# Tomiinek/Multilingual_Text_to_Speech

Measured on NVIDIA H100. Metric: mel-frames/sec (train fwd+bwd), higher is better.
Workload: dtype bf16

## Files before the change

### multilingual_text_to_speech_b200/csrc/decoder_persist_bwd.cu

```cuda
#include <cuda_bf16.h>
#include "decoder_internal.cuh"
#include "tc_ptx.cuh"

namespace b200tts {

namespace {

constexpr int PT = 256;

__device__ __forceinline__ void ldmatrix_x4(uint32_t& r0, uint32_t& r1, uint32_t& r2, uint32_t& r3, const void* p) {
    const uint32_t addr = (uint32_t)__cvta_generic_to_shared(p);
    asm volatile("ldmatrix.sync.aligned.m8n8.x4.shared.b16 {%0,%1,%2,%3}, [%4];\n" : "=r"(r0), "=r"(r1), "=r"(r2), "=r"(r3) : "r"(addr));
}
__device__ __forceinline__ void mma_bf16(float (&c)[4], const uint32_t (&a)[4], uint32_t b0, uint32_t b1) {
    asm volatile("mma.sync.aligned.m16n8k16.row.col.f32.bf16.bf16.f32 {%0,%1,%2,%3}, {%4,%5,%6,%7}, {%8,%9}, {%0,%1,%2,%3};\n"
                 : "+f"(c[0]), "+f"(c[1]), "+f"(c[2]), "+f"(c[3])
                 : "r"(a[0]), "r"(a[1]), "r"(a[2]), "r"(a[3]), "r"(b0), "r"(b1));
}
struct NoOverlap { __device__ __forceinline__ void operator()() const {} };
template <typename Overlap = NoOverlap>
__device__ __forceinline__ bool grid_barrier(unsigned* counter, unsigned& target, unsigned nblocks, int* abort_flag, bool async_fence = false,
                                             Overlap overlap = Overlap()) {
    __shared__ int s_ok;
    __syncthreads();
    if (threadIdx.x == 0) {
        target += nblocks;
        if (async_fence) tcx::proxy_fence_global();
        asm volatile("red.release.gpu.global.add.u32 [%0], 1;" ::"l"(counter) : "memory");
    }
    overlap();
    if (threadIdx.x == 0) {
        int ok = 1;
        const long long t0 = clock64();
        unsigned polls = 0;
        for (;;) {
            unsigned v;
            asm volatile("ld.relaxed.gpu.global.u32 %0, [%1];" : "=r"(v) : "l"(counter) : "memory");
            if (v >= target) break;
            if ((++polls & 255u) == 0 && (clock64() - t0 > 4000000000ll || *reinterpret_cast<volatile int*>(abort_flag))) {
                ok = 0; *abort_flag = 1; break;
            }
        }
        asm volatile("fence.acquire.gpu;" ::: "memory");
        s_ok = ok;
    }
    __syncthreads();
    return s_ok != 0;
}

__device__ __forceinline__ void l2_prefetch(const void* p) { asm volatile("prefetch.global.L2 [%0];" ::"l"(p)); }
__device__ __forceinline__ void cp_async16(void* smem, const void* gmem) {
    asm volatile("cp.async.cg.shared.global [%0], [%1], 16;" ::"r"((uint32_t)__cvta_generic_to_shared(smem)), "l"(gmem) : "memory");
}
__device__ __forceinline__ void cp_async8(void* smem, const void* gmem) {
    asm volatile("cp.async.ca.shared.global [%0], [%1], 8;" ::"r"((uint32_t)__cvta_generic_to_shared(smem)), "l"(gmem) : "memory");
}
__device__ __forceinline__ void cp_async_wait_all() { asm volatile("cp.async.wait_all;" ::: "memory"); }
__device__ __forceinline__ void st_async_peer_f32(const float* local_smem, const uint64_t* local_bar, uint32_t peer_rank, float v) {
    uint32_t ra, rb;
    asm volatile("mapa.shared::cluster.u32 %0, %1, %2;" : "=r"(ra) : "r"((uint32_t)__cvta_generic_to_shared(local_smem)), "r"(peer_rank));
    asm volatile("mapa.shared::cluster.u32 %0, %1, %2;" : "=r"(rb) : "r"((uint32_t)__cvta_generic_to_shared(local_bar)), "r"(peer_rank));
    asm volatile("st.async.shared::cluster.mbarrier::complete_tx::bytes.b32 [%0], %1, [%2];" ::"r"(ra), "r"(__float_as_uint(v)), "r"(rb) : "memory");
}
__device__ __forceinline__ float tanh_exp(float x) { return 2.f * __fdividef(1.f, 1.f + __expf(-2.f * x)) - 1.f; }

#define BPROF_DECL long long prof_acc[8] = {0, 0, 0, 0, 0, 0, 0, 0}; long long prof_t = clock64();
#define BPROF_MARK(slot)                                                                                         \
    do {                                                                                                         \
        if (p.prof && threadIdx.x == 0) { const long long now = clock64(); prof_acc[slot] += now - prof_t; prof_t = now; } \
    } while (0)
#define BPROF_FLUSH                                                                                              \
    do {                                                                                                         \
        if (p.prof && threadIdx.x == 0)                                                                          \
            for (int k9 = 0; k9 < 8; ++k9) p.prof[(size_t)blockIdx.x * 8 + k9] = prof_acc[k9];                   \
    } while (0)

constexpr int KBA = 8;
constexpr int GLD = 33;
constexpr int NBT = 16;
constexpr int TUN = 80;
constexpr int TUN_WIDE = 96;

struct AttBwdArgs {
    int B, T, D, M, L, A, KC, NOUT, UK, UN, MT;
    const float* W; int ldw;
    const float* gates; const float* cstate;
    const float* dh_static;
    const float* dctx_static;
    const uint8_t* mask_h; const uint8_t* mask_c;
    int kind, training; float rate_h, rate_c;
    float* dgates;
    __nv_bfloat16* dgb;
    long long dgb_step; int dgb_rows;
    float* part;
    const float* q; const float* cum; const float* align; long long align_bstride;
    const float* dalign; long long dalign_bstride;
    const float* bias; const float* v; const float* Wq;
    const __nv_bfloat16* WcB;
    const __nv_bfloat16* WcB2;
    const __nv_bfloat16* memTf;
    const uint4* memFb; int M16;
    const int* lengths;
    float* dctx_tot;
    float* dq;
    float* de;
    unsigned* barrier; int* abort_flag;
    long long* prof;
};

__device__ __forceinline__ uint32_t pack2(float lo, float hi) {
    __nv_bfloat162 v = __floats2bfloat162_rn(lo, hi);
    return *reinterpret_cast<uint32_t*>(&v);
}
__device__ __forceinline__ float tanh_fast(float x) {
    float y;
    asm("tanh.approx.f32 %0, %1;" : "=f"(y) : "f"(x));
    return y;
}

template <int UNC>
__global__ void __launch_bounds__(PT, 1) att_bwd_loop_kernel(const __grid_constant__ CUtensorMap tmG, const AttBwdArgs p) {
    extern __shared__ __align__(1024) unsigned char smem_raw0[];
    unsigned char* smem_raw = reinterpret_cast<unsigned char*>((reinterpret_cast<uintptr_t>(smem_raw0) + 1023) & ~(uintptr_t)1023);
    __shared__ uint64_t full_bar[2], xb1, xb2;
    const int tid = threadIdx.x, lane = tid & 31, warp = tid >> 5;
    const int cta = blockIdx.x;
    const int kb = (cta >> 1) % KBA, nb = 2 * (cta >> 4) + (cta & 1);
    const int B = p.B, D = p.D, UK = p.UK, UN = p.UN, KROWS = 4 * UK, M = p.M, L = p.L, A = p.A;
    const int n0 = nb * UN;
    const int NKT = KROWS / 64;
    unsigned char* sW = smem_raw;
    __nv_bfloat16* As = reinterpret_cast<__nv_bfloat16*>(smem_raw + (size_t)NKT * UN * 128);
    unsigned char* extra = reinterpret_cast<unsigned char*>(As) + (size_t)NKT * 8192;
    __nv_bfloat16* sWcB = reinterpret_cast<__nv_bfloat16*>(extra);
    __nv_bfloat16* sWcB2 = sWcB + (size_t)A * 40;
    float* dcum = reinterpret_cast<float*>(sWcB2 + (size_t)32 * (A + 8));
    uint4* wqf = reinterpret_cast<uint4*>(dcum + (p.MT * 16 + 32));
    float* s_dhq = reinterpret_cast<float*>(wqf + (size_t)(A / 16) * 32);
    float* s_pbo = s_dhq + 2 * 64 * 8;
    uint8_t* s_pbm = reinterpret_cast<uint8_t*>(s_pbo + (size_t)6 * B * 8);
    float* s_rp = reinterpret_cast<float*>(s_pbm + (size_t)2 * B * 8);
    const unsigned nblocks = gridDim.x;
    const int L16 = p.MT * 16;

    for (int idx = tid; idx < KROWS * UN; idx += PT) {
        const int r = idx / UN, n = idx % UN;
        const int g = r / UK, uk = r % UK;
        float w = 0.f;
        if (n0 + n < p.NOUT) w = p.W[(size_t)(g * D + kb * UK + uk) * p.ldw + n0 + n];
        const int c = r >> 6, kc = r & 63;
        *reinterpret_cast<__nv_bfloat16*>(sW + (size_t)c * UN * 128 + n * 128 + ((((kc >> 3) ^ (n & 7))) << 4) + (kc & 7) * 2) = __float2bfloat16_rn(w);
    }
    for (int idx = tid; idx < A * 40; idx += PT) sWcB[idx] = p.WcB[idx];
    for (int idx = tid; idx < 32 * (A + 8); idx += PT) sWcB2[idx] = p.WcB2[idx];
    for (int idx = tid; idx < L16 + 32; idx += PT) dcum[idx] = 0.f;
    const int UOWN = 8;
    const bool owner = cta * UOWN < D;
    const int uo0 = cta * UOWN;
    if (owner)
        for (int idx = tid; idx < (A / 16) * 32; idx += PT) {
            const int kk = idx >> 5, g = (idx >> 2) & 7, tq = idx & 3;
            uint32_t f[4];
#pragma unroll
            for (int r2 = 0; r2 < 2; ++r2) {
                const int a = kk * 16 + 2 * tq + 8 * r2;
                const float x0 = p.Wq[(size_t)a * D + uo0 + g], x1 = p.Wq[(size_t)(a + 1) * D + uo0 + g];
                const __nv_bfloat16 h0 = __float2bfloat16_rn(x0), h1 = __float2bfloat16_rn(x1);
                __nv_bfloat162 hp; hp.x = h0; hp.y = h1;
                f[r2] = *reinterpret_cast<uint32_t*>(&hp);
                f[2 + r2] = pack2(x0 - __bfloat162float(h0), x1 - __bfloat162float(h1));
            }
            wqf[idx] = make_uint4(f[0], f[1], f[2], f[3]);
        }
    uint32_t prod_it = 0;
    if (tid == 0) { tcx::mbar_init(&xb1, 1); tcx::mbar_init(&xb2, 1); tcx::mbar_init_fence(); }
    if (tid == 0) { tcx::mbar_init(&full_bar[0], 1); tcx::mbar_init(&full_bar[1], 1); tcx::mbar_init_fence(); }
    tcx::proxy_fence_shared();
    __syncthreads();
    tcx::cluster_arrive(); tcx::cluster_wait();

    const float inv_h = 1.f / (1.f - p.rate_h), inv_c = 1.f / (1.f - p.rate_c);
    constexpr int MAXE = 3;
    float dc_reg[MAXE], dhz_reg[MAXE];
#pragma unroll
    for (int e = 0; e < MAXE; ++e) { dc_reg[e] = 0.f; dhz_reg[e] = 0.f; }
    unsigned target = 0;

    float* scr = reinterpret_cast<float*>(As);
    float* s_dctx = scr;
    float* s_w = s_dctx + ((M + 3) & ~3);
    float* s_de = s_w + L16;
    float* s_qb = s_de + L16;
    float* s_vv = s_qb + A;
    uint32_t* s_Ph = reinterpret_cast<uint32_t*>(s_vv + A);
    uint32_t* s_Pl = s_Ph + (L16 + 48);
    float* s_red = reinterpret_cast<float*>(s_Pl + (L16 + 48));
    const int hf = cta & 1, HT0 = (p.MT + 1) / 2;
    const int t_lo = hf ? HT0 : 0, t_hi = hf ? p.MT : HT0;
    const int g_lo = hf ? (HT0 - 1) * 16 : 0;
    float* s_G = s_red + 64;
    float* s_dqp = s_G + (size_t)(HT0 + 1) * 16 * GLD;
    float* s_dqx = s_dqp + 8 * A;
    float* s_dotx = s_dqx + A;
    float* s_stage = s_dotx + 4;
    uint2* s_bf = reinterpret_cast<uint2*>(s_stage + L16);
    BPROF_DECL

    const int pc = cta >> 1;
    auto pb_stage = [&](int step) {
        if (!owner || step < 0) return;
        const size_t row = (size_t)step * B;
        for (int c = tid; c < 12 * B; c += PT) {
            const int k = c / (2 * B), r = c - k * 2 * B, b = r >> 1, h4 = (r & 1) * 4;
            const float* src = k < 4 ? p.gates + (row + b) * 4 * D + (size_t)k * D : (k == 4 ? p.cstate : p.dh_static) + (row + b) * D;
            cp_async16(s_pbo + (k * B + b) * UOWN + h4, src + uo0 + h4);
        }
        if (p.training)
            for (int c = tid; c < 2 * B; c += PT) {
                const int k = c / B, b = c - k * B;
                const uint8_t* m = k ? p.mask_c : p.mask_h;
                if (m) cp_async8(s_pbm + (k * B + b) * UOWN, m + (row + b) * D + uo0);
            }
// ... 58 lines not shown
                    }
                    if (m < L16) { s_w[m] = r_w[e]; s_de[m] = r_da[e]; }
                    if (m < L16 + 48) {
                        const __nv_bfloat16 h0 = __float2bfloat16_rn(r_c0[e]), h1 = __float2bfloat16_rn(r_c1[e]);
                        __nv_bfloat162 hp; hp.x = h0; hp.y = h1;
                        s_Ph[m] = *reinterpret_cast<uint32_t*>(&hp);
                        s_Pl[m] = pack2(r_c0[e] - __bfloat162float(h0), r_c1[e] - __bfloat162float(h1));
                    }
                }
                if (tid < A) { s_qb[tid] = r_q + bias_r; s_vv[tid] = v_r; }
            }
            __syncthreads();
            for (int idx = tid; idx < p.M16 * 32; idx += PT) {
                const int kt = idx >> 5, gg = (idx >> 2) & 7, tt = idx & 3;
                const int m0 = kt * 16 + 2 * tt;
                uint2 f = make_uint2(0u, 0u);
                if (gg < 2) {
                    const float w0 = m0 < M ? s_dctx[m0] : 0.f, w1 = m0 + 1 < M ? s_dctx[m0 + 1] : 0.f;
                    const float w2 = m0 + 8 < M ? s_dctx[m0 + 8] : 0.f, w3 = m0 + 9 < M ? s_dctx[m0 + 9] : 0.f;
                    const float h0 = __bfloat162float(__float2bfloat16_rn(w0)), h1 = __bfloat162float(__float2bfloat16_rn(w1));
                    const float h2 = __bfloat162float(__float2bfloat16_rn(w2)), h3 = __bfloat162float(__float2bfloat16_rn(w3));
                    f = gg == 0 ? make_uint2(pack2(h0, h1), pack2(h2, h3)) : make_uint2(pack2(w0 - h0, w1 - h1), pack2(w2 - h2, w3 - h3));
                }
                s_bf[idx] = f;
            }
            __syncthreads();
            {
                const int g = lane >> 2, tq = lane & 3;
                for (int lt = t_lo + warp; lt < t_hi; lt += 8) {
                    float dacc[4] = {0.f, 0.f, 0.f, 0.f}, dacc2[4] = {0.f, 0.f, 0.f, 0.f};
                    if (lt * 16 < len) {
                        const uint4* fr = p.memFb + (((size_t)b * p.MT + lt) * p.M16) * 32 + lane;
                        for (int kt0 = 0; kt0 < p.M16; kt0 += KT) {
                            uint4 av[KT];
#pragma unroll
                            for (int j = 0; j < KT; ++j)
                                if (kt0 + j < p.M16) av[j] = __ldg(fr + (size_t)(kt0 + j) * 32);
                            uint32_t bfr[KT][2];
#pragma unroll
                            for (int j = 0; j < KT; ++j) {
                                bfr[j][0] = 0u; bfr[j][1] = 0u;
                                if (kt0 + j < p.M16) { const uint2 f = s_bf[(kt0 + j) * 32 + lane]; bfr[j][0] = f.x; bfr[j][1] = f.y; }
                            }
#pragma unroll
                            for (int j = 0; j < KT; j += 2) {
                                if (kt0 + j < p.M16) {
                                    const uint32_t af[4] = {av[j].x, av[j].y, av[j].z, av[j].w};
                                    mma_bf16(dacc, af, bfr[j][0], bfr[j][1]);
                                }
                                if (kt0 + j + 1 < p.M16) {
                                    const uint32_t af[4] = {av[j + 1].x, av[j + 1].y, av[j + 1].z, av[j + 1].w};
                                    mma_bf16(dacc2, af, bfr[j + 1][0], bfr[j + 1][1]);
                                }
                            }
                        }
                    }
#pragma unroll
                    for (int q4 = 0; q4 < 4; ++q4) dacc[q4] += dacc2[q4];
                    if (tq == 0) {
#pragma unroll
                        for (int rr = 0; rr < 2; ++rr) {
                            const int l = lt * 16 + g + 8 * rr;
                            float gv = 0.f;
                            if (l < len) gv = (rr ? dacc[2] + dacc[3] : dacc[0] + dacc[1]) + (last ? 0.f : dcum[l]) + s_de[l];
                            s_de[l] = gv;
                        }
                    }
                }
            }
            __syncthreads();
            float pdot = 0.f;
            for (int l = t_lo * 16 + tid; l < t_hi * 16 && l < len; l += PT) pdot = fmaf(s_w[l], s_de[l], pdot);
            pdot = block_sum(pdot, s_red);
            if (tid == 0) { tcx::mbar_expect_tx(&xb1, 4); st_async_peer_f32(s_dotx, &xb1, (uint32_t)(hf ^ 1), pdot); }
            tcx::mbar_wait(&xb1, (uint32_t)(p.T - 1 - i) & 1);
            const float dot = pdot + s_dotx[0];
            for (int l = t_lo * 16 + tid; l < t_hi * 16; l += PT) {
                const float d = l < len ? s_w[l] * (s_de[l] - dot) : 0.f;
                s_de[l] = d;
                if (l < L) p.de[((size_t)i * B + b) * L + l] = d;
            }
            __syncthreads();
            BPROF_MARK(0);
            float dqacc[16][2];
#pragma unroll
            for (int nt = 0; nt < 16; ++nt) { dqacc[nt][0] = 0.f; dqacc[nt][1] = 0.f; }
            const int g = lane >> 2, tq = lane & 3;
            for (int mt = t_lo + warp; mt < t_hi && mt < mtiles; mt += 8) {
                const int l0 = mt * 16;
                float sacc[16][4];
#pragma unroll
                for (int nt = 0; nt < 16; ++nt)
#pragma unroll
                    for (int e = 0; e < 4; ++e) sacc[nt][e] = 0.f;
#pragma unroll
                for (int ks = 0; ks < 2; ++ks) {
                    const int x = l0 + ks * 16 + g + 2 * tq;
                    uint32_t ah[4], al[4];
                    ah[0] = s_Ph[x]; ah[1] = s_Ph[x + 8]; ah[2] = s_Ph[x + 8]; ah[3] = s_Ph[x + 16];
                    al[0] = s_Pl[x]; al[1] = s_Pl[x + 8]; al[2] = s_Pl[x + 8]; al[3] = s_Pl[x + 16];
#pragma unroll
                    for (int np = 0; np < 8; ++np) {
                        uint32_t bf[4];
                        ldmatrix_x4(bf[0], bf[1], bf[2], bf[3], sWcB + (size_t)(np * 16 + (lane & 7) + ((lane >> 4) << 3)) * 40 + ks * 16 + ((lane >> 3) & 1) * 8);
                        mma_bf16(sacc[2 * np], ah, bf[0], bf[1]);
                        mma_bf16(sacc[2 * np], al, bf[0], bf[1]);
                        mma_bf16(sacc[2 * np + 1], ah, bf[2], bf[3]);
                        mma_bf16(sacc[2 * np + 1], al, bf[2], bf[3]);
                    }
                }
                const uint4* mf = reinterpret_cast<const uint4*>(p.memTf + (((size_t)b * p.MT + mt) * 32 + lane) * 64);
                const float de0 = s_de[l0 + g], de1 = s_de[l0 + g + 8];
                uint32_t dsA[16][2];
#pragma unroll
                for (int c4 = 0; c4 < 8; ++c4) {
                    const uint4 raw = mf[c4];
                    const uint32_t words[4] = {raw.x, raw.y, raw.z, raw.w};
#pragma unroll
                    for (int hf = 0; hf < 2; ++hf) {
                        const int nt = 2 * c4 + hf;
                        const float2 m01 = __bfloat1622float2(*reinterpret_cast<const __nv_bfloat162*>(&words[2 * hf]));
                        const float2 m23 = __bfloat1622float2(*reinterpret_cast<const __nv_bfloat162*>(&words[2 * hf + 1]));
                        const int a0 = nt * 8 + 2 * tq;
                        const float t0 = tanh_fast(sacc[nt][0] + s_qb[a0] + m01.x), t1 = tanh_fast(sacc[nt][1] + s_qb[a0 + 1] + m01.y);
                        const float t2 = tanh_fast(sacc[nt][2] + s_qb[a0] + m23.x), t3 = tanh_fast(sacc[nt][3] + s_qb[a0 + 1] + m23.y);
                        const float d0 = de0 * s_vv[a0] * (1.f - t0 * t0), d1 = de0 * s_vv[a0 + 1] * (1.f - t1 * t1);
                        const float d2 = de1 * s_vv[a0] * (1.f - t2 * t2), d3 = de1 * s_vv[a0 + 1] * (1.f - t3 * t3);
                        dqacc[nt][0] += d0 + d2; dqacc[nt][1] += d1 + d3;
                        dsA[nt][0] = pack2(d0, d1); dsA[nt][1] = pack2(d2, d3);
                    }
                }
                float gacc[4][4];
#pragma unroll
                for (int nt = 0; nt < 4; ++nt)
#pragma unroll
                    for (int e = 0; e < 4; ++e) gacc[nt][e] = 0.f;
#pragma unroll
                for (int j = 0; j < 8; ++j) {
                    const uint32_t af[4] = {dsA[2 * j][0], dsA[2 * j][1], dsA[2 * j + 1][0], dsA[2 * j + 1][1]};
#pragma unroll
                    for (int np = 0; np < 2; ++np) {
                        uint32_t bf[4];
                        ldmatrix_x4(bf[0], bf[1], bf[2], bf[3], sWcB2 + (size_t)(np * 16 + (lane & 7) + ((lane >> 4) << 3)) * (A + 8) + j * 16 + ((lane >> 3) & 1) * 8);
                        mma_bf16(gacc[2 * np], af, bf[0], bf[1]);
                        mma_bf16(gacc[2 * np + 1], af, bf[2], bf[3]);
                    }
                }
#pragma unroll
                for (int nt = 0; nt < 4; ++nt)
#pragma unroll
                    for (int e = 0; e < 4; ++e) s_G[(l0 - g_lo + g + 8 * (e >> 1)) * GLD + nt * 8 + 2 * tq + (e & 1)] = gacc[nt][e];
            }
            tcx::proxy_fence_shared();
            __syncthreads();
            {
                const int ht = hf ? HT0 : HT0 - 1;
                const int peer_g_lo = hf ? 0 : (HT0 - 1) * 16;
                if (tid == 0 && ht >= t_lo && ht < t_hi)
                    tcx::bulk_copy_to_peer(s_G + (size_t)(ht * 16 - peer_g_lo) * GLD, s_G + (size_t)(ht * 16 - g_lo) * GLD, 16 * GLD * 4, &xb2,
                                           (uint32_t)(hf ^ 1));
            }
#pragma unroll
            for (int nt = 0; nt < 16; ++nt)
#pragma unroll
                for (int c = 0; c < 2; ++c) {
                    float v = dqacc[nt][c];
                    v += __shfl_xor_sync(0xffffffffu, v, 4);
                    v += __shfl_xor_sync(0xffffffffu, v, 8);
                    v += __shfl_xor_sync(0xffffffffu, v, 16);
                    if (g == 0) s_dqp[warp * A + nt * 8 + 2 * tq + c] = v;
                }
            __syncthreads();
            float pdq = 0.f;
            if (tid < A) {
#pragma unroll
                for (int w8 = 0; w8 < 8; ++w8) pdq += s_dqp[w8 * A + tid];
                st_async_peer_f32(s_dqx + tid, &xb2, (uint32_t)(hf ^ 1), pdq);
            }
            {
                const bool peer_sends_tile = hf ? true : (HT0 < p.MT);
                if (tid == 0) tcx::mbar_expect_tx(&xb2, (uint32_t)(A * 4 + (peer_sends_tile ? 16 * GLD * 4 : 0)));
            }
            tcx::mbar_wait(&xb2, (uint32_t)(p.T - 1 - i) & 1);
            if (hf == 0 && tid < A) p.dq[((size_t)i * B + b) * A + tid] = pdq + s_dqx[tid];
            for (int j = t_lo * 16 + tid; j < t_hi * 16 && j < L; j += PT) {
                float acc = last ? 0.f : dcum[j];
#pragma unroll 4
                for (int k = 0; k < p.KC; ++k) {
                    const int l = j + half - k;
                    if (l >= 0 && l < mtiles * 16) acc += s_G[(size_t)(l - g_lo) * GLD + k];
                }
                s_stage[j] = acc;
            }
            __syncthreads();
            for (int j = t_lo * 16 + tid; j < t_hi * 16 && j < L; j += PT) dcum[j] = s_stage[j];
        }
        BPROF_MARK(1);
        if (!grid_barrier(p.barrier, target, nblocks, p.abort_flag)) break;
        BPROF_MARK(2);

        if (owner) {
            float* s_dq = reinterpret_cast<float*>(As);
            if (!last)
                for (int c = tid; c < KBA * B * 2; c += PT) {
                    const int kb2 = c >> 1, h4 = (c & 1) * 4;
                    cp_async16(s_rp + kb2 * UOWN + h4, p.part + (size_t)kb2 * p.NOUT + M + uo0 + h4);
                }
            {
                const float4* dq4 = reinterpret_cast<const float4*>(p.dq + (size_t)i * B * A);
                for (int idx = tid; idx < B * 32; idx += PT) {
                    const int b = idx >> 5, c4 = idx & 31;
                    cp_async16(s_dq + b * A + ((c4 * 4 + 8 * (b & 7)) & (A - 1)), dq4 + idx);
                }
            }
            cp_async_wait_all();
            __syncthreads();
            float rec_[MAXE];
#pragma unroll
            for (int e = 0; e < MAXE; ++e) {
                const int idx = tid + e * PT;
                float rs = 0.f;
                if (idx < B * UOWN && !last) {
#pragma unroll
                    for (int k2 = 0; k2 < KBA; ++k2) rs += s_rp[k2 * B * UOWN + idx];
                }
                rec_[e] = rs;
            }
            {
                const int g = lane >> 2, tq = lane & 3, mt = warp & 3, kh = warp >> 2;
                float acc[4] = {0.f, 0.f, 0.f, 0.f};
                const int ksteps = A / 32;
#pragma unroll 4
                for (int ks = 0; ks < ksteps; ++ks) {
                    const int a0 = (kh * ksteps + ks) * 16;
                    uint32_t ah[4], al[4];
#pragma unroll
                    for (int r4 = 0; r4 < 4; ++r4) {
                        const int br = mt * 16 + g + 8 * (r4 & 1);
                        const float2 x = *reinterpret_cast<const float2*>(s_dq + br * A + ((a0 + 2 * tq + 8 * (r4 >> 1) + 8 * (br & 7)) & (A - 1)));
                        const __nv_bfloat16 h0 = __float2bfloat16_rn(x.x), h1 = __float2bfloat16_rn(x.y);
                        __nv_bfloat162 hp; hp.x = h0; hp.y = h1;
                        ah[r4] = *reinterpret_cast<uint32_t*>(&hp);
                        al[r4] = pack2(x.x - __bfloat162float(h0), x.y - __bfloat162float(h1));
                    }
                    const uint4 wf = wqf[(a0 >> 4) * 32 + lane];
                    mma_bf16(acc, ah, wf.x, wf.y);
                    mma_bf16(acc, al, wf.x, wf.y);
                    mma_bf16(acc, ah, wf.z, wf.w);
                }
                float* d0 = s_dhq + ((kh * 64) + mt * 16 + g) * UOWN + 2 * tq;
                float* d1 = d0 + 8 * UOWN;
                d0[0] = acc[0]; d0[1] = acc[1]; d1[0] = acc[2]; d1[1] = acc[3];
                __syncthreads();
            }
#pragma unroll
// ... 256 lines not shown

__global__ void att_bwd_prep_kernel(__nv_bfloat16* __restrict__ WcB, __nv_bfloat16* __restrict__ WcB2, __nv_bfloat16* __restrict__ memTf,
                                    const float* __restrict__ WcombT, const float* __restrict__ memT, int B, int L, int A, int KC, int MT) {
    const size_t n1 = (size_t)A * 40, n2 = (size_t)32 * (A + 8), n3 = (size_t)B * MT * 32 * 64;
    for (size_t idx = blockIdx.x * (size_t)blockDim.x + threadIdx.x; idx < n1 + n2 + n3; idx += (size_t)gridDim.x * blockDim.x) {
        if (idx < n1) {
            const int a = idx / 40, k = idx % 40;
            WcB[idx] = __float2bfloat16_rn(k < KC ? WcombT[(size_t)k * A + a] : 0.f);
        } else if (idx < n1 + n2) {
            const size_t j = idx - n1;
            const int k = j / (A + 8), a = j % (A + 8);
            WcB2[j] = __float2bfloat16_rn((k < KC && a < A) ? WcombT[(size_t)k * A + a] : 0.f);
        } else {
            const size_t j = idx - n1 - n2;
            const int v = j % 64, lane = (j / 64) % 32, mt = (j / (64 * 32)) % MT, b = j / ((size_t)64 * 32 * MT);
            const int nt = v / 4, e = v % 4, g = lane >> 2, tq = lane & 3;
            const int l = mt * 16 + g + 8 * (e >> 1), a = nt * 8 + 2 * tq + (e & 1);
            memTf[j] = __float2bfloat16_rn((l < L && a < A) ? memT[((size_t)b * L + l) * A + a] : 0.f);
        }
    }
}

__global__ void att_bwd_reduce_parts_kernel(float* __restrict__ dWsum, float* __restrict__ dvsum, const float* __restrict__ dWcomb_part,
                                            const float* __restrict__ dv_part, int nparts, int A) {
    const int idx = blockIdx.x * blockDim.x + threadIdx.x;
    if (idx < A * 32) {
        float s0 = 0.f, s1 = 0.f, s2 = 0.f, s3 = 0.f;
        int p2 = 0;
        for (; p2 + 3 < nparts; p2 += 4) {
            s0 += dWcomb_part[(size_t)p2 * A * 32 + idx]; s1 += dWcomb_part[(size_t)(p2 + 1) * A * 32 + idx];
            s2 += dWcomb_part[(size_t)(p2 + 2) * A * 32 + idx]; s3 += dWcomb_part[(size_t)(p2 + 3) * A * 32 + idx];
        }
        for (; p2 < nparts; ++p2) s0 += dWcomb_part[(size_t)p2 * A * 32 + idx];
        dWsum[idx] = (s0 + s1) + (s2 + s3);
    } else if (idx < A * 32 + A) {
        const int a = idx - A * 32;
        float sv = 0.f;
        for (int p2 = 0; p2 < nparts; ++p2) sv += dv_part[(size_t)p2 * A + a];
        dvsum[a] = sv;
    }
}
__global__ void att_bwd_finish_kernel(float* __restrict__ dWloc, float* __restrict__ dWc, float* __restrict__ dv,
                                      const float* __restrict__ dWsum, const float* __restrict__ dvsum,
                                      const float* __restrict__ Wloc, const float* __restrict__ Wc, int A, int C, int KC) {
    extern __shared__ float dW[];
    for (int idx = threadIdx.x; idx < A * 32; idx += blockDim.x) dW[idx] = dWsum[idx];
    for (int a = threadIdx.x; a < A; a += blockDim.x) dv[a] += dvsum[a];
    __syncthreads();
    for (int idx = threadIdx.x; idx < A * C; idx += blockDim.x) {
        const int a = idx / C, c = idx % C;
        float s = 0.f;
        for (int k = 0; k < KC; ++k) s = fmaf(dW[a * 32 + k], Wc[c * KC + k], s);
        dWloc[idx] += s;
    }
    for (int idx = threadIdx.x; idx < C * KC; idx += blockDim.x) {
        const int c = idx / KC, k = idx % KC;
        float s = 0.f;
        for (int a = 0; a < A; ++a) s = fmaf(Wloc[a * C + c], dW[a * 32 + k], s);
        dWc[idx] += s;
    }
}

}

AttBwdExtra att_bwd_extra(const b200tts_decoder_shape& s) {
    AttBwdExtra x;
    size_t off = 0;
    auto take = [&](size_t n) { size_t o = off; off = (off + n + 255) / 256 * 256; return o; };
    x.MT = (s.L + 15) / 16;
    x.part = take((size_t)KBA * s.B * (s.M + s.D) * 4);
    x.wcb = take((size_t)s.A * 40 * 2);
    x.wcb2 = take((size_t)32 * (s.A + 8) * 2);
    x.memTf = take((size_t)s.B * x.MT * 32 * 64 * 2);
    x.de = take((size_t)s.T * s.B * s.L * 4);
    x.dwpart = take((size_t)s.B * x.MT * s.A * 32 * 4);
    x.dvpart = take((size_t)s.B * x.MT * s.A * 4);
    x.barrier = take(256 + NUM_SMS * 8 * 8);
    x.total = off;
    return x;
}

struct AttBwdGeom {
    int UK, UN, grid; size_t region, smem;
};
static AttBwdGeom att_bwd_geom(const b200tts_decoder_shape& s) {
    AttBwdGeom g{};
    g.UK = s.D / KBA;
    const int L16 = (s.L + 15) / 16 * 16;
    const size_t extras = (size_t)s.A * 40 * 2 + (size_t)32 * (s.A + 8) * 2 + (size_t)(L16 + 32) * 4 + (size_t)s.A * 32 + 2 * 64 * 8 * 4 +
                          (size_t)s.B * 8 * (6 * 4 + 2 + KBA * 4);
    g.UN = (s.M + s.D <= NBT * TUN) ? TUN : TUN_WIDE; g.grid = KBA * NBT;
    const int NKT = 4 * g.UK / 64;
    g.region = (size_t)NKT * 8192;
    g.smem = 1024 + (size_t)NKT * g.UN * 128 + g.region + extras;
    return g;
}

bool persist_att_bwd_supported(const b200tts_decoder_shape& s) {
    const AttBwdGeom g = att_bwd_geom(s);
    if (s.A != 128 || s.K > 32 || s.B * 8 > 3 * PT || s.D % KBA != 0) return false;
    if (s.M > 2 * PT || (s.L + 15) / 16 * 16 + 48 > 2 * PT) return false;
    if (s.D / 8 > g.grid) return false;
    if (g.grid / 2 < s.B || g.grid > NUM_SMS) return false;
    if (g.UK % 64 != 0 || s.B > 64 || s.M + s.D > NBT * g.UN || (s.M + s.D) % 4 != 0) return false;
    const int MT = (s.L + 15) / 16, L16 = MT * 16, HT0 = (MT + 1) / 2;
    const size_t fl = (size_t)((s.M + 3) & ~3) + 3 * (size_t)L16 + 2 * s.A + 2 * (size_t)(L16 + 48) + 64 + (size_t)(HT0 + 1) * 16 * GLD +
                      8 * (size_t)s.A + s.A + 4 + (size_t)((s.M + 15) / 16) * 32 * 2;
    if (fl * 4 > g.region) return false;
    if ((size_t)s.B * s.A * 4 + 64 * 8 * 4 > g.region) return false;
    return g.smem <= 227 * 1024;
}

int tc_make_mapN_bf16(void* map, const void* base, int rank, const unsigned long long* dims, const unsigned long long* strides, const unsigned* box);

int persist_att_bwd_loop(const b200tts_decoder_shape& s, const b200tts_decoder_params& w, const b200tts_decoder_inputs& in,
                         const DecoderLayout& fl, const float* fws, const PersistLayout& pl, const unsigned char* pws,
                         const float* align, const float* dalign, const float* dh_static, const float* dctx_static, float* dgates,
                         float* dq, float* dctx_tot, float* dmemT, unsigned char* extra, const b200tts_decoder_params& dw,
                         cudaStream_t st, void* dgb_hist) {
    const AttBwdExtra x = att_bwd_extra(s);
    const int B = s.B, D = s.D, M = s.M, T = s.T, L = s.L, A = s.A;
    B200_REQUIRE(persist_att_bwd_supported(s), "persistent attention backward: shape not supported");
    const AttBwdGeom geo = att_bwd_geom(s);
    B200_REQUIRE(!s.training || ((uintptr_t)in.mask_att_h | (uintptr_t)in.mask_att_c) % 8 == 0,
                 "persistent attention backward: the attention-LSTM keep masks must be 8-byte aligned");
    AttBwdArgs a{};
    a.B = B; a.T = T; a.D = D; a.M = M; a.L = L; a.A = A; a.KC = s.K; a.NOUT = M + D; a.UK = geo.UK;
    a.UN = geo.UN; a.MT = x.MT;
    a.W = fws + fl.wcat_att; a.ldw = M + D;
    a.gates = fws + fl.ga; a.cstate = fws + fl.ca; a.dh_static = dh_static; a.dctx_static = dctx_static;
    a.mask_h = in.mask_att_h; a.mask_c = in.mask_att_c; a.kind = s.cell_kind; a.training = s.training; a.rate_h = s.rate_h; a.rate_c = s.rate_c;
    a.dgates = dgates;
    a.dgb = static_cast<__nv_bfloat16*>(dgb_hist); a.dgb_step = (long long)B * 4 * D; a.dgb_rows = B;
    a.part = reinterpret_cast<float*>(extra + x.part);
    a.q = fws + fl.q; a.cum = fws + fl.cum; a.align = align; a.align_bstride = (long long)T * L;
    a.dalign = dalign; a.dalign_bstride = (long long)T * L;
    a.bias = w.attn_bias; a.v = w.attn_energy; a.Wq = w.attn_query;
    __nv_bfloat16* wcb = reinterpret_cast<__nv_bfloat16*>(extra + x.wcb);
    __nv_bfloat16* wcb2 = reinterpret_cast<__nv_bfloat16*>(extra + x.wcb2);
    __nv_bfloat16* memTf = reinterpret_cast<__nv_bfloat16*>(extra + x.memTf);
    a.WcB = wcb; a.WcB2 = wcb2; a.memTf = memTf;
    a.memFb = reinterpret_cast<const uint4*>(pws + pl.memFb); a.M16 = pl.M16;
    a.lengths = in.text_lengths; a.dctx_tot = dctx_tot; a.dq = dq; a.de = reinterpret_cast<float*>(extra + x.de);
    a.barrier = reinterpret_cast<unsigned*>(extra + x.barrier); a.abort_flag = reinterpret_cast<int*>(a.barrier + 32);
    a.prof = reinterpret_cast<long long*>(extra + x.barrier + 256);
    const float* wcombT = reinterpret_cast<const float*>(pws + pl.wcombT);
    B200_CUDA(cudaMemsetAsync(a.barrier, 0, 256, st));
    att_bwd_prep_kernel<<<NUM_SMS * 4, 256, 0, st>>>(wcb, wcb2, memTf, wcombT, fws + fl.memT, B, L, A, s.K, x.MT);
    B200_LAUNCH_CHECK();
    const size_t smem = geo.smem;
    void* fn = geo.UN == TUN ? (void*)att_bwd_loop_kernel<TUN> : (void*)att_bwd_loop_kernel<TUN_WIDE>;
    B200_CUDA(cudaFuncSetAttribute(fn, cudaFuncAttributeMaxDynamicSharedMemorySize, (int)smem));
    const int grid = geo.grid;
    int per_sm = 0, dev = 0, sms = 0;
    B200_CUDA(cudaOccupancyMaxActiveBlocksPerMultiprocessor(&per_sm, fn, PT, smem));
    B200_CUDA(cudaGetDevice(&dev));
    B200_CUDA(cudaDeviceGetAttribute(&sms, cudaDevAttrMultiProcessorCount, dev));
    B200_REQUIRE(per_sm * sms >= grid && grid % 2 == 0 && grid / 2 >= B, "persistent attention backward: %d CTAs cannot be co-resident / paired", grid);
    CUtensorMap tm;
    const unsigned long long dims[5] = {64ull, (unsigned long long)T * B, (unsigned long long)(geo.UK / 64), (unsigned long long)KBA, 4ull};
    const unsigned long long strides[4] = {(unsigned long long)4 * D * 2, 128ull, (unsigned long long)geo.UK * 2, (unsigned long long)D * 2};
    const unsigned box[5] = {64u, 64u, (unsigned)(geo.UK / 64), 1u, 2u};
    B200_TRY(tc_make_mapN_bf16(&tm, a.dgb, 5, dims, strides, box));
    void* params[] = {&tm, &a};
    cudaLaunchConfig_t cfg{};
    cfg.gridDim = dim3(grid); cfg.blockDim = dim3(PT); cfg.dynamicSmemBytes = smem; cfg.stream = st;
    cudaLaunchAttribute attrs[2];
    attrs[0].id = cudaLaunchAttributeCooperative;
    attrs[0].val.cooperative = 1;
    attrs[1].id = cudaLaunchAttributeClusterDimension;
    attrs[1].val.clusterDim.x = 2; attrs[1].val.clusterDim.y = 1; attrs[1].val.clusterDim.z = 1;
    cfg.attrs = attrs; cfg.numAttrs = 2;
    int nclusters = 0;
    B200_CUDA(cudaOccupancyMaxActiveClusters(&nclusters, fn, &cfg));
    B200_REQUIRE(nclusters * 2 >= grid, "persistent attention backward: only %d CTA pairs can be co-resident, %d needed", nclusters, grid / 2);
    {
        KernelTimer kt("att_bwd_loop_kernel", st);
        B200_CUDA(cudaLaunchKernelExC(&cfg, fn, params));
    }
    B200_LAUNCH_CHECK();
    AttPostArgs pp{};
    pp.B = B; pp.T = T; pp.L = L; pp.A = A; pp.KC = s.K; pp.MT = x.MT;
    pp.q = a.q; pp.cum = a.cum; pp.de = a.de; pp.bias = w.attn_bias; pp.v = w.attn_energy; pp.WcB = wcb; pp.memT = fws + fl.memT;
    pp.lengths = in.text_lengths; pp.dmemT = dmemT;
    pp.dWcomb_part = reinterpret_cast<float*>(extra + x.dwpart); pp.dv_part = reinterpret_cast<float*>(extra + x.dvpart);
    B200_CUDA(cudaMemsetAsync(dmemT, 0, (size_t)B * L * A * 4, st));
    B200_CUDA(cudaMemsetAsync(pp.dWcomb_part, 0, (size_t)B * x.MT * A * 32 * 4, st));
    B200_CUDA(cudaMemsetAsync(pp.dv_part, 0, (size_t)B * x.MT * A * 4, st));
    {
        KernelTimer kt("att_post_kernel", st);
        att_post_kernel<<<B * x.MT, PT, 0, st>>>(pp);
    }
    B200_LAUNCH_CHECK();
    float* dWsum = a.de;
    float* dvsum = dWsum + (size_t)A * 32;
    att_bwd_reduce_parts_kernel<<<cdiv(A * 32 + A, 128), 128, 0, st>>>(dWsum, dvsum, pp.dWcomb_part, pp.dv_part, B * x.MT, A);
    B200_LAUNCH_CHECK();
    att_bwd_finish_kernel<<<1, 512, (size_t)A * 32 * 4, st>>>(dw.attn_location, dw.attn_loc_features, dw.attn_energy, dWsum, dvsum,
                                                             w.attn_location, w.attn_loc_features, A, s.C, s.K);
    B200_LAUNCH_CHECK();
    return B200TTS_OK;
}

}
```

Before: 736,800.

## Split attention-backward energy tiles across warp quarters and stage dS through shared memory

Restructures the per-step location-attention backward inner loop. Before, each warp owned whole 16-row tiles and computed all 128 attention columns. Now each warp handles a quarter of the attention columns (q = warp&3) for several tiles, and prefetches the next memT fragment from global memory. The bf16 dS tiles are written to spare shared memory in the As region, and after a barrier a second pass runs the WcB2 GEMM with B fragments kept in registers. The goal is lower register pressure, better latency hiding and reuse of the WcB2 fragments, at the cost of extra shared-memory traffic, extra __syncthreads, and more complex slot/geometry bookkeeping.

Result: no change. 743,900 (median of 6 runs) (+1.0%).

```diff
diff --git a/multilingual_text_to_speech_b200/csrc/decoder_persist_bwd.cu b/multilingual_text_to_speech_b200/csrc/decoder_persist_bwd.cu
--- a/multilingual_text_to_speech_b200/csrc/decoder_persist_bwd.cu
+++ b/multilingual_text_to_speech_b200/csrc/decoder_persist_bwd.cu
@@ -101,6 +101,7 @@
     const __nv_bfloat16* memTf;
     const uint4* memFb; int M16;
     const int* lengths;
+    int ds_off, ds_slots;
     float* dctx_tot;
     float* dq;
     float* de;
@@ -132,12 +133,12 @@
     unsigned char* sW = smem_raw;
     __nv_bfloat16* As = reinterpret_cast<__nv_bfloat16*>(smem_raw + (size_t)NKT * UN * 128);
     unsigned char* extra = reinterpret_cast<unsigned char*>(As) + (size_t)NKT * 8192;
-    __nv_bfloat16* sWcB = reinterpret_cast<__nv_bfloat16*>(extra);
+    float* s_dhq = reinterpret_cast<float*>(extra);
+    __nv_bfloat16* sWcB = reinterpret_cast<__nv_bfloat16*>(s_dhq + 2 * 64 * 8);
     __nv_bfloat16* sWcB2 = sWcB + (size_t)A * 40;
     float* dcum = reinterpret_cast<float*>(sWcB2 + (size_t)32 * (A + 8));
     uint4* wqf = reinterpret_cast<uint4*>(dcum + (p.MT * 16 + 32));
-    float* s_dhq = reinterpret_cast<float*>(wqf + (size_t)(A / 16) * 32);
-    float* s_pbo = s_dhq + 2 * 64 * 8;
+    float* s_pbo = reinterpret_cast<float*>(wqf + (size_t)(A / 16) * 32);
     uint8_t* s_pbm = reinterpret_cast<uint8_t*>(s_pbo + (size_t)6 * B * 8);
     float* s_rp = reinterpret_cast<float*>(s_pbm + (size_t)2 * B * 8);
     const unsigned nblocks = gridDim.x;
@@ -362,74 +363,117 @@
             }
             __syncthreads();
             BPROF_MARK(0);
-            float dqacc[16][2];
-#pragma unroll
-            for (int nt = 0; nt < 16; ++nt) { dqacc[nt][0] = 0.f; dqacc[nt][1] = 0.f; }
-            const int g = lane >> 2, tq = lane & 3;
-            for (int mt = t_lo + warp; mt < t_hi && mt < mtiles; mt += 8) {
-                const int l0 = mt * 16;
-                float sacc[16][4];
-#pragma unroll
-                for (int nt = 0; nt < 16; ++nt)
-#pragma unroll
-                    for (int e = 0; e < 4; ++e) sacc[nt][e] = 0.f;
-#pragma unroll
-                for (int ks = 0; ks < 2; ++ks) {
-                    const int x = l0 + ks * 16 + g + 2 * tq;
-                    uint32_t ah[4], al[4];
-                    ah[0] = s_Ph[x]; ah[1] = s_Ph[x + 8]; ah[2] = s_Ph[x + 8]; ah[3] = s_Ph[x + 16];
-                    al[0] = s_Pl[x]; al[1] = s_Pl[x + 8]; al[2] = s_Pl[x + 8]; al[3] = s_Pl[x + 16];
-#pragma unroll
-                    for (int np = 0; np < 8; ++np) {
-                        uint32_t bf[4];
-                        ldmatrix_x4(bf[0], bf[1], bf[2], bf[3], sWcB + (size_t)(np * 16 + (lane & 7) + ((lane >> 4) << 3)) * 40 + ks * 16 + ((lane >> 3) & 1) * 8);
-                        mma_bf16(sacc[2 * np], ah, bf[0], bf[1]);
-                        mma_bf16(sacc[2 * np], al, bf[0], bf[1]);
-                        mma_bf16(sacc[2 * np + 1], ah, bf[2], bf[3]);
-                        mma_bf16(sacc[2 * np + 1], al, bf[2], bf[3]);
-                    }
-                }
-                const uint4* mf = reinterpret_cast<const uint4*>(p.memTf + (((size_t)b * p.MT + mt) * 32 + lane) * 64);
-                const float de0 = s_de[l0 + g], de1 = s_de[l0 + g + 8];
-                uint32_t dsA[16][2];
-#pragma unroll
-                for (int c4 = 0; c4 < 8; ++c4) {
-                    const uint4 raw = mf[c4];
-                    const uint32_t words[4] = {raw.x, raw.y, raw.z, raw.w};
-#pragma unroll
-                    for (int hf = 0; hf < 2; ++hf) {
-                        const int nt = 2 * c4 + hf;
-                        const float2 m01 = __bfloat1622float2(*reinterpret_cast<const __nv_bfloat162*>(&words[2 * hf]));
-                        const float2 m23 = __bfloat1622float2(*reinterpret_cast<const __nv_bfloat162*>(&words[2 * hf + 1]));
-                        const int a0 = nt * 8 + 2 * tq;
-                        const float t0 = tanh_fast(sacc[nt][0] + s_qb[a0] + m01.x), t1 = tanh_fast(sacc[nt][1] + s_qb[a0 + 1] + m01.y);
-                        const float t2 = tanh_fast(sacc[nt][2] + s_qb[a0] + m23.x), t3 = tanh_fast(sacc[nt][3] + s_qb[a0 + 1] + m23.y);
-                        const float d0 = de0 * s_vv[a0] * (1.f - t0 * t0), d1 = de0 * s_vv[a0 + 1] * (1.f - t1 * t1);
-                        const float d2 = de1 * s_vv[a0] * (1.f - t2 * t2), d3 = de1 * s_vv[a0 + 1] * (1.f - t3 * t3);
-                        dqacc[nt][0] += d0 + d2; dqacc[nt][1] += d1 + d3;
-                        dsA[nt][0] = pack2(d0, d1); dsA[nt][1] = pack2(d2, d3);
-                    }
-                }
-                float gacc[4][4];
-#pragma unroll
-                for (int nt = 0; nt < 4; ++nt)
-#pragma unroll
-                    for (int e = 0; e < 4; ++e) gacc[nt][e] = 0.f;
-#pragma unroll
-                for (int j = 0; j < 8; ++j) {
-                    const uint32_t af[4] = {dsA[2 * j][0], dsA[2 * j][1], dsA[2 * j + 1][0], dsA[2 * j + 1][1]};
-#pragma unroll
-                    for (int np = 0; np < 2; ++np) {
-                        uint32_t bf[4];
-                        ldmatrix_x4(bf[0], bf[1], bf[2], bf[3], sWcB2 + (size_t)(np * 16 + (lane & 7) + ((lane >> 4) << 3)) * (A + 8) + j * 16 + ((lane >> 3) & 1) * 8);
-                        mma_bf16(gacc[2 * np], af, bf[0], bf[1]);
-                        mma_bf16(gacc[2 * np + 1], af, bf[2], bf[3]);
-                    }
-                }
-#pragma unroll
-                for (int nt = 0; nt < 4; ++nt)
-#pragma unroll
-                    for (int e = 0; e < 4; ++e) s_G[(l0 - g_lo + g + 8 * (e >> 1)) * GLD + nt * 8 + 2 * tq + (e & 1)] = gacc[nt][e];
+            const int g = lane >> 2, tq = lane & 3, q = warp & 3;
+            const int nown = max(0, min(t_hi, mtiles) - t_lo);
+            uint4* s_ds = reinterpret_cast<uint4*>(reinterpret_cast<unsigned char*>(As) + p.ds_off);
+            for (int s0 = 0; s0 < 8; s0 += p.ds_slots) {
+                const int s1 = min(s0 + p.ds_slots, 8);
+                const int n1 = max(0, min(s1, nown) - s0), n2 = max(0, min(s1, nown - 8) - s0);
+                uint4 nraw[2];
+                auto load_memT = [&](int k) {
+                    const uint4* mf = reinterpret_cast<const uint4*>(p.memTf + (((size_t)b * p.MT + t_lo + k) * 32 + lane) * 64) + 2 * q;
+                    nraw[0] = __ldg(mf); nraw[1] = __ldg(mf + 1);
+                };
+                if (s0 + (warp >> 2) < min(s1, nown)) load_memT(s0 + (warp >> 2));
+                for (int s = s0 + (warp >> 2); s < s1; s += 2) {
+                    float dqacc[4][2];
+#pragma unroll
+                    for (int nt = 0; nt < 4; ++nt) { dqacc[nt][0] = 0.f; dqacc[nt][1] = 0.f; }
+                    for (int k = s; k < nown; k += 8) {
+                        const int l0 = (t_lo + k) * 16;
+                        const uint4 raw[2] = {nraw[0], nraw[1]};
+                        const int nk = k + 8 < nown ? k + 8 : (s + 2 < s1 ? s + 2 : nown);
+                        if (nk < nown) load_memT(nk);
+                        float sacc[4][4];
+#pragma unroll
+                        for (int nt = 0; nt < 4; ++nt)
+#pragma unroll
+                            for (int e = 0; e < 4; ++e) sacc[nt][e] = 0.f;
+#pragma unroll
+                        for (int ks = 0; ks < 2; ++ks) {
+                            const int x = l0 + ks * 16 + g + 2 * tq;
+                            uint32_t ah[4], al[4];
+                            ah[0] = s_Ph[x]; ah[1] = s_Ph[x + 8]; ah[2] = s_Ph[x + 8]; ah[3] = s_Ph[x + 16];
+                            al[0] = s_Pl[x]; al[1] = s_Pl[x + 8]; al[2] = s_Pl[x + 8]; al[3] = s_Pl[x + 16];
+#pragma unroll
+                            for (int np = 0; np < 2; ++np) {
+                                uint32_t bf[4];
+                                ldmatrix_x4(bf[0], bf[1], bf[2], bf[3],
+                                            sWcB + (size_t)((2 * q + np) * 16 + (lane & 7) + ((lane >> 4) << 3)) * 40 + ks * 16 + ((lane >> 3) & 1) * 8);
+                                mma_bf16(sacc[2 * np], ah, bf[0], bf[1]);
+                                mma_bf16(sacc[2 * np], al, bf[0], bf[1]);
+                                mma_bf16(sacc[2 * np + 1], ah, bf[2], bf[3]);
+                                mma_bf16(sacc[2 * np + 1], al, bf[2], bf[3]);
+                            }
+                        }
+                        const float de0 = s_de[l0 + g], de1 = s_de[l0 + g + 8];
+                        uint4* dst = s_ds + (k < 8 ? k - s0 : n1 + k - 8 - s0) * 256 + lane;
+#pragma unroll
+                        for (int c4 = 0; c4 < 2; ++c4) {
+                            const uint32_t words[4] = {raw[c4].x, raw[c4].y, raw[c4].z, raw[c4].w};
+                            uint32_t af[4];
+#pragma unroll
+                            for (int h2 = 0; h2 < 2; ++h2) {
+                                const int nt = 2 * c4 + h2, ntg = 4 * q + nt;
+                                const float2 m01 = __bfloat1622float2(*reinterpret_cast<const __nv_bfloat162*>(&words[2 * h2]));
+                                const float2 m23 = __bfloat1622float2(*reinterpret_cast<const __nv_bfloat162*>(&words[2 * h2 + 1]));
+                                const int a0 = ntg * 8 + 2 * tq;
+                                const float t0 = tanh_fast(sacc[nt][0] + s_qb[a0] + m01.x), t1 = tanh_fast(sacc[nt][1] + s_qb[a0 + 1] + m01.y);
+                                const float t2 = tanh_fast(sacc[nt][2] + s_qb[a0] + m23.x), t3 = tanh_fast(sacc[nt][3] + s_qb[a0 + 1] + m23.y);
+                                const float d0 = de0 * s_vv[a0] * (1.f - t0 * t0), d1 = de0 * s_vv[a0 + 1] * (1.f - t1 * t1);
+                                const float d2 = de1 * s_vv[a0] * (1.f - t2 * t2), d3 = de1 * s_vv[a0 + 1] * (1.f - t3 * t3);
+                                dqacc[nt][0] += d0 + d2; dqacc[nt][1] += d1 + d3;
+                                af[2 * h2] = pack2(d0, d1); af[2 * h2 + 1] = pack2(d2, d3);
+                            }
+                            dst[(2 * q + c4) * 32] = make_uint4(af[0], af[1], af[2], af[3]);
+                        }
+                    }
+#pragma unroll
+                    for (int nt = 0; nt < 4; ++nt)
+#pragma unroll
+                        for (int c = 0; c < 2; ++c) {
+                            float v = dqacc[nt][c];
+                            v += __shfl_xor_sync(0xffffffffu, v, 4);
+                            v += __shfl_xor_sync(0xffffffffu, v, 8);
+                            v += __shfl_xor_sync(0xffffffffu, v, 16);
+                            if (g == 0) s_dqp[s * A + (4 * q + nt) * 8 + 2 * tq + c] = v;
+                        }
+                }
+                __syncthreads();
+                const int nst = n1 + n2;
+                if ((warp >> 2) < nst) {
+                    uint32_t wb[8][2];
+#pragma unroll
+                    for (int jp = 0; jp < 4; ++jp)
+                        ldmatrix_x4(wb[2 * jp][0], wb[2 * jp][1], wb[2 * jp + 1][0], wb[2 * jp + 1][1],
+                                    sWcB2 + (size_t)(q * 8 + (lane & 7)) * (A + 8) + (2 * jp + (lane >> 4)) * 16 + ((lane >> 3) & 1) * 8);
+                    for (int b0 = warp >> 2; b0 < nst; b0 += 8) {
+                        float gacc[4][4];
+#pragma unroll
+                        for (int m = 0; m < 4; ++m)
+#pragma unroll
+                            for (int e = 0; e < 4; ++e) gacc[m][e] = 0.f;
+#pragma unroll
+                        for (int j = 0; j < 8; ++j)
+#pragma unroll
+                            for (int m = 0; m < 4; ++m)
+                                if (b0 + 2 * m < nst) {
+                                    const uint4 a4 = s_ds[(b0 + 2 * m) * 256 + j * 32 + lane];
+                                    const uint32_t af[4] = {a4.x, a4.y, a4.z, a4.w};
+                                    mma_bf16(gacc[m], af, wb[j][0], wb[j][1]);
+                                }
+#pragma unroll
+                        for (int m = 0; m < 4; ++m) {
+                            const int bi = b0 + 2 * m;
+                            if (bi < nst) {
+                                const int l0 = (t_lo + (bi < n1 ? s0 + bi : s0 + bi - n1 + 8)) * 16;
+#pragma unroll
+                                for (int e = 0; e < 4; ++e) s_G[(l0 - g_lo + g + 8 * (e >> 1)) * GLD + q * 8 + 2 * tq + (e & 1)] = gacc[m][e];
+                            }
+                        }
+                    }
+                }
+                if (s1 < 8) __syncthreads();
             }
             tcx::proxy_fence_shared();
             __syncthreads();
@@ -440,17 +484,6 @@
                     tcx::bulk_copy_to_peer(s_G + (size_t)(ht * 16 - peer_g_lo) * GLD, s_G + (size_t)(ht * 16 - g_lo) * GLD, 16 * GLD * 4, &xb2,
                                            (uint32_t)(hf ^ 1));
             }
-#pragma unroll
-            for (int nt = 0; nt < 16; ++nt)
-#pragma unroll
-                for (int c = 0; c < 2; ++c) {
-                    float v = dqacc[nt][c];
-                    v += __shfl_xor_sync(0xffffffffu, v, 4);
-                    v += __shfl_xor_sync(0xffffffffu, v, 8);
-                    v += __shfl_xor_sync(0xffffffffu, v, 16);
-                    if (g == 0) s_dqp[warp * A + nt * 8 + 2 * tq + c] = v;
-                }
-            __syncthreads();
             float pdq = 0.f;
             if (tid < A) {
 #pragma unroll
@@ -873,17 +906,23 @@
 
 struct AttBwdGeom {
     int UK, UN, grid; size_t region, smem;
+    size_t scratch;
+    int ds_tiles, ds_slots;
 };
 static AttBwdGeom att_bwd_geom(const b200tts_decoder_shape& s) {
     AttBwdGeom g{};
     g.UK = s.D / KBA;
-    const int L16 = (s.L + 15) / 16 * 16;
+    const int MT = (s.L + 15) / 16, L16 = MT * 16, HT0 = (MT + 1) / 2;
     const size_t extras = (size_t)s.A * 40 * 2 + (size_t)32 * (s.A + 8) * 2 + (size_t)(L16 + 32) * 4 + (size_t)s.A * 32 + 2 * 64 * 8 * 4 +
                           (size_t)s.B * 8 * (6 * 4 + 2 + KBA * 4);
     g.UN = (s.M + s.D <= NBT * TUN) ? TUN : TUN_WIDE; g.grid = KBA * NBT;
     const int NKT = 4 * g.UK / 64;
     g.region = (size_t)NKT * 8192;
     g.smem = 1024 + (size_t)NKT * g.UN * 128 + g.region + extras;
+    g.scratch = 4 * ((size_t)((s.M + 3) & ~3) + 3 * (size_t)L16 + 2 * s.A + 2 * (size_t)(L16 + 48) + 64 + (size_t)(HT0 + 1) * 16 * GLD +
+                     8 * (size_t)s.A + s.A + 4 + (size_t)((s.M + 15) / 16) * 32 * 2);
+    g.ds_tiles = g.scratch <= g.region ? (int)((g.region + 4096 - g.scratch) / 4096) : 0;
+    g.ds_slots = g.ds_tiles >= HT0 ? 8 : g.ds_tiles / (HT0 > 8 ? 2 : 1);
     return g;
 }
 
@@ -894,10 +933,7 @@
     if (s.D / 8 > g.grid) return false;
     if (g.grid / 2 < s.B || g.grid > NUM_SMS) return false;
     if (g.UK % 64 != 0 || s.B > 64 || s.M + s.D > NBT * g.UN || (s.M + s.D) % 4 != 0) return false;
-    const int MT = (s.L + 15) / 16, L16 = MT * 16, HT0 = (MT + 1) / 2;
-    const size_t fl = (size_t)((s.M + 3) & ~3) + 3 * (size_t)L16 + 2 * s.A + 2 * (size_t)(L16 + 48) + 64 + (size_t)(HT0 + 1) * 16 * GLD +
-                      8 * (size_t)s.A + s.A + 4 + (size_t)((s.M + 15) / 16) * 32 * 2;
-    if (fl * 4 > g.region) return false;
+    if (g.scratch > g.region || g.ds_slots < 1) return false;
     if ((size_t)s.B * s.A * 4 + 64 * 8 * 4 > g.region) return false;
     return g.smem <= 227 * 1024;
 }
@@ -932,7 +968,9 @@
     __nv_bfloat16* memTf = reinterpret_cast<__nv_bfloat16*>(extra + x.memTf);
     a.WcB = wcb; a.WcB2 = wcb2; a.memTf = memTf;
     a.memFb = reinterpret_cast<const uint4*>(pws + pl.memFb); a.M16 = pl.M16;
-    a.lengths = in.text_lengths; a.dctx_tot = dctx_tot; a.dq = dq; a.de = reinterpret_cast<float*>(extra + x.de);
+    a.lengths = in.text_lengths;
+    a.ds_off = (int)(geo.region + 4096 - (size_t)geo.ds_tiles * 4096); a.ds_slots = geo.ds_slots;
+    a.dctx_tot = dctx_tot; a.dq = dq; a.de = reinterpret_cast<float*>(extra + x.de);
     a.barrier = reinterpret_cast<unsigned*>(extra + x.barrier); a.abort_flag = reinterpret_cast<int*>(a.barrier + 32);
     a.prof = reinterpret_cast<long long*>(extra + x.barrier + 256);
     const float* wcombT = reinterpret_cast<const float*>(pws + pl.wcombT);
```
